# ParBLiSS/FastANI

Measured on NVIDIA H100. Metric: genome-pairs/sec (many-to-many, k=16, fragLen=3000), higher is better.
Workload: dtype u64

## Files before the change

### fastani_b200/csrc/map.cu

```cuda
#include "common.cuh"
#include "cgi_rows.hpp"
#include <algorithm>
#include <cstring>
#include <deque>

namespace bani {

static inline unsigned nblk(uint64_t n, int t = 256) { return (unsigned)((n + t - 1) / t); }

static constexpr int SU_THREADS = 128;
static constexpr int SU_CAP = 4096;

__global__ void __launch_bounds__(SU_THREADS)
sort_unique_kernel(uint32_t *fragHash, const uint32_t *segStart, int32_t F, int32_t *sCount,
                   int *smax, int *err, int minN )
{
  __shared__ uint32_t a[SU_CAP];
  __shared__ uint32_t wsum[SU_THREADS / 32];
  const int f = blockIdx.x, tid = threadIdx.x;
  const uint32_t beg = segStart[f];
  const int n = (int)(segStart[f + 1] - beg);
  if (n <= minN) return;
  if (n > SU_CAP) { if (tid == 0) { atomicExch(err, 1); sCount[f] = 0; } return; }
  if (n == 0) { if (tid == 0) sCount[f] = 0; return; }
// ... 160 lines not shown
  if (i > fragBeg) {
    const uint32_t rp = (uint32_t)a.keys[i - 1]; int32_t sp;
    if (a.recSeq[rp] == a.recSeq[ra] && l1_qual(a, i - 1, fragEnd, mh, rp, sp) && a.recWpos[rp] >= start) merged = true;
  }
  if (!merged) fl |= 1;
  bool nextMerges = false;
  if (i + 1 < fragEnd) {
    const uint32_t rn = (uint32_t)a.keys[i + 1]; int32_t sn;
    if (a.recSeq[rn] == a.recSeq[ra] && l1_qual(a, i + 1, fragEnd, mh, rn, sn) && a.recWpos[ra] >= sn) nextMerges = true;
  }
  if (!nextMerges) fl |= 2;
  return fl;
}

__global__ void l1_flag_kernel(const L1Args a, uint32_t *head)
{
  unsigned long long i = (unsigned long long)blockIdx.x * blockDim.x + threadIdx.x;
  if (i > a.N) return;
  if (i == a.N) { head[i] = 0; return; }
  int32_t start; uint32_t ra; int f;
  head[i] = l1_flags(a, i, start, ra, f) & 1u;
}

__global__ void l1_write_kernel(const L1Args a, const uint32_t *head, const uint32_t *headScan,
                                int32_t *cFrag, int32_t *cSeq, int32_t *cStart, int32_t *cEnd)
{
  unsigned long long i = (unsigned long long)blockIdx.x * blockDim.x + threadIdx.x;
  if (i >= a.N) return;
  int32_t start; uint32_t ra; int f;
  const uint32_t fl = l1_flags(a, i, start, ra, f);
  if (fl & 1) { const uint32_t c = headScan[i]; cFrag[c] = f; cSeq[c] = a.recSeq[ra]; cStart[c] = start; }
  if (fl & 2) { const uint32_t c = headScan[i] + head[i] - 1; cEnd[c] = a.recWpos[ra]; }
}

struct L2Args {
  const int32_t *cFrag, *cSeq, *cStart, *cEnd; uint32_t C;
  const uint32_t *fragHash; const uint32_t *segStart; const int32_t *sCount;
  const uint32_t *recHash; const int32_t *recWpos; const uint32_t *recLink; const uint32_t *contigRecOff;
  int fragLen, cmw, smax;
  uint8_t *scratch; size_t stride;
  int32_t *cPos, *cBest;
  int onlyFlagged;
};

__device__ __forceinline__ uint32_t lb_wpos(const int32_t *wpos, uint32_t lo, uint32_t hi, int32_t v)
{
  while (lo < hi) { uint32_t mid = (lo + hi) >> 1; if (wpos[mid] < v) lo = mid + 1; else hi = mid; }
  return lo;
}
__device__ __forceinline__ int lb_q(const uint32_t *Q, int s, uint32_t h)
{
  int lo = 0, hi = s;
  while (lo < hi) { int mid = (lo + hi) >> 1; if (Q[mid] < h) lo = mid + 1; else hi = mid; }
  return lo;
}

__global__ void __launch_bounds__(64)
l2_kernel(const L2Args a)
{
  const uint32_t slot = blockIdx.x * blockDim.x + threadIdx.x, nslots = gridDim.x * blockDim.x;
  uint16_t *gap = (uint16_t *)(a.scratch + (size_t)slot * a.stride);
  uint8_t *pres = (uint8_t *)(gap + a.smax + 2);
  for (uint32_t c = slot; c < a.C; c += nslots) {
    if (a.onlyFlagged && a.cBest[c] != -1) continue;
    const int f = a.cFrag[c];
    const int s = a.sCount[f];
    const uint32_t *Q = a.fragHash + a.segStart[f];
    const int seq = a.cSeq[c];
    const uint32_t lo = a.contigRecOff[seq], hi = a.contigRecOff[seq + 1];
    uint32_t b = lb_wpos(a.recWpos, lo, hi, a.cStart[c]);
    uint32_t e = lb_wpos(a.recWpos, lo, hi, a.recWpos[b] + a.cmw);
    const uint32_t last = lb_wpos(a.recWpos, lo, hi, a.cEnd[c] + a.fragLen);
    for (int i = 0; i <= s; i++) gap[i] = 0;
    for (int i = 0; i < s; i++) pres[i] = 0;
    int t = s, G = 0, P = 0;

    auto insert = [&](uint32_t r, uint32_t wb) {
      const uint32_t pd = a.recLink[r] >> 16;
      if (pd != 0xFFFFu && r - pd >= wb) return;
      const uint32_t h = a.recHash[r];
      const int j = lb_q(Q, s, h);
      if (j < s && Q[j] == h) { pres[j] = 1; if (j < t) P++; }
      else { gap[j]++; if (j < t) G++; while (t + G > s) { t--; G -= gap[t]; P -= pres[t]; } }
    };
    auto remove = [&](uint32_t r, uint32_t we) {
      const uint32_t nd = a.recLink[r] & 0xFFFFu;
      if (nd != 0xFFFFu && r + nd < we) return;
      const uint32_t h = a.recHash[r];
      const int j = lb_q(Q, s, h);
      if (j < s && Q[j] == h) { pres[j] = 0; if (j < t) P--; }
      else { gap[j]--; if (j < t) G--; while (t < s && t + 1 + G + (int)gap[t] <= s) { G += gap[t]; P += pres[t]; t++; } }
    };

    for (uint32_t r = b; r < e; r++) insert(r, b);
    int sw = a.recWpos[b];
    int best = 0, first = 0, lastp = 0;
    while (e < last) {
      if (P > best) { best = P; first = lastp = a.recWpos[b]; }
      else if (P == best) lastp = a.recWpos[b];
      const int d1 = a.recWpos[b + 1] - sw, d2 = a.recWpos[e] - (sw + a.cmw - 1);
      const int adv = min(d1, d2);
      sw += adv;
      const uint32_t ob = b, oe = e;
      if (adv == d1) { remove(ob, oe); b++; }
      if (adv == d2) { insert(oe, b); e++; }
    }
    a.cPos[c] = (first + lastp) / 2;
    a.cBest[c] = best;
  }
}

static constexpr int L2_SMAX = 2047;
static constexpr int L2_SHM_BUDGET = 200 * 1024;
static constexpr uint32_t EV_M = 1u, EV_D = 2u, EV_S = 4u, EV_JMASK = 0xFFE0u;
__host__ __device__ __forceinline__ uint32_t ev_rank(uint32_t j) { return j << 5; }

static constexpr int L2E_RING = 1024;
static constexpr int L2E_FLUSH_IT = 4;
static constexpr int L2E_BF_MAX = L2E_RING - 64 * L2E_FLUSH_IT - 96;

struct L2PArgs {
  const int32_t *cFrag, *cSeq, *cStart, *cEnd; uint32_t C;
  const uint32_t *fragCandOff;
  const uint32_t *fragHash; const uint32_t *segStart; const int32_t *sCount;
  const uint4 *rec; const int32_t *recWposSoA; const uint32_t *contigRecOff;
  const uint2 *rec8; const uint32_t *recLink; const uint32_t *blkMax;
  int fragLen, cmw, sLimit, shiftA, nBuckets;
  int stage;
  uint32_t *cB0, *cE0, *cLast, *cNEv, *cChunks;
  uint16_t *cMB;
  const uint32_t *cOff;
  const unsigned long long *grpOff;
  uint16_t *events;
  const uint32_t *perm; uint32_t warpBytes;
  int32_t *cPos, *cBest; unsigned long long *ctr_n2;
};

__global__ void frag_cand_off_kernel(const int32_t *cFrag, uint32_t C, int32_t F, uint32_t *fragCandOff)
{
  int f = blockIdx.x * blockDim.x + threadIdx.x;
  if (f > F) return;
  uint32_t lo = 0, hi = C;
  while (lo < hi) { uint32_t mid = (lo + hi) >> 1; if (cFrag[mid] < f) lo = mid + 1; else hi = mid; }
  fragCandOff[f] = lo;
}

__device__ __forceinline__ int32_t rec_wpos(const uint4 *rec, uint32_t i) { return (int32_t)(__ldg(&rec[i].y) & 0x7FFFFFFFu); }
__device__ __forceinline__ uint32_t lb_rec(const uint4 *rec, uint32_t lo, uint32_t hi, int32_t v)
{
  while (lo < hi) { uint32_t mid = (lo + hi) >> 1; if (rec_wpos(rec, mid) < v) lo = mid + 1; else hi = mid; }
  return lo;
}

__global__ void l2_bounds_kernel(const L2PArgs a)
{
  const uint32_t c = blockIdx.x * blockDim.x + threadIdx.x;
  unsigned long long n2 = 0;
  if (c < a.C) {
    const int seq = a.cSeq[c];
    const uint32_t lo = a.contigRecOff[seq], hi = a.contigRecOff[seq + 1];
    const uint32_t b0 = lb_wpos(a.recWposSoA, lo, hi, a.cStart[c]);
    const uint32_t e0 = lb_wpos(a.recWposSoA, b0, hi, __ldg(&a.recWposSoA[b0]) + a.cmw);
    const uint32_t last = lb_wpos(a.recWposSoA, b0, hi, a.cEnd[c] + a.fragLen);
    n2 = last - b0;
    const int s = a.sCount[a.cFrag[c]];
    uint32_t nEv = 0;
    if (e0 < last) {
      const uint32_t back = __ldg(&a.rec[last - 1].w) & 0xFFFFu;
      const uint32_t bEnd = (back > last - 1 - b0) ? b0 : last - 1 - back;
      nEv = (e0 - b0) + (last - e0) + (bEnd - b0);
    }
    a.cB0[c] = b0; a.cE0[c] = e0; a.cLast[c] = last;
    const bool fast = s >= 1 && s <= a.sLimit && nEv < (1u << 20);
    {
      uint32_t mbk = 0, mfw = 0;
      if (fast && nEv) {
        const uint32_t blk1 = (last - 1) >> 10;
        for (uint32_t blk = b0 >> 10; blk <= blk1 && mbk != 0xFFFFu; blk++) { const uint32_t v = __ldg(&a.blkMax[blk]); mbk = max(mbk, v & 0xFFFFu); mfw = max(mfw, v >> 16); }
      }
      a.cMB[c] = (uint16_t)((a.stage && mbk + mfw <= (uint32_t)L2E_BF_MAX) ? mbk : 0xFFFFu);
    }
    a.cNEv[c] = fast ? nEv : 0u;
    a.cChunks[c] = fast ? (nEv + 15) >> 4 : 0u;
    a.cBest[c] = (fast || nEv == 0) ? 0 : -1;
    a.cPos[c] = 0;
  } else if (c == a.C) a.cChunks[c] = 0;
  for (int o = 16; o; o >>= 1) n2 += __shfl_xor_sync(0xffffffffu, n2, o);
  if ((threadIdx.x & 31) == 0 && n2) atomicAdd(a.ctr_n2, n2);
}

__global__ void l2_sortkey_kernel(const uint32_t *cNEv, uint32_t C, uint32_t *key, uint32_t *val)
{
  const uint32_t c = blockIdx.x * blockDim.x + threadIdx.x;
  if (c >= C) return;
  key[c] = 0xFFFFFu - min(cNEv[c], 0xFFFFFu);
  val[c] = c;
}

__global__ void l2_group_steps_kernel(const uint32_t *cChunks, const uint32_t *perm, uint32_t C, uint32_t nGrp, uint32_t *grpSteps)
{
  const uint32_t G = blockIdx.x * blockDim.x + threadIdx.x;
  if (G > nGrp) return;
  grpSteps[G] = G < nGrp ? cChunks[perm[G * 32]] : 0u;
}
__global__ void l2_stream_base_kernel(const uint32_t *perm, const unsigned long long *grpOff, uint32_t C, uint32_t *cOff)
{
  const uint32_t g = blockIdx.x * blockDim.x + threadIdx.x;
  if (g >= C) return;
  cOff[perm[g]] = (uint32_t)(grpOff[g >> 5] * 32ull + (g & 31u));
}
__device__ __forceinline__ size_t ev_index(uint32_t base, uint32_t e) { return ((size_t)base + (size_t)(e >> 4) * 32) * 16 + (e & 15u); }

static constexpr int L2E_BUCKETS = 4096;

template <int NT>
__global__ void __launch_bounds__(NT)
l2_events_kernel(const L2PArgs a)
{
  extern __shared__ __align__(16) uint32_t smem[];
  __shared__ uint32_t s_wsum[NT / 32];
  constexpr int NW = NT / 32;
  const int f = blockIdx.x, tid = threadIdx.x, lane = tid & 31, wid = tid >> 5;
  const uint32_t c0 = a.fragCandOff[f], c1 = a.fragCandOff[f + 1];
  if (c0 == c1) return;
  const int s = a.sCount[f];
  if (s < 1 || s > a.sLimit) return;
  uint16_t *ring = reinterpret_cast<uint16_t *>(smem) + wid * L2E_RING;
  uint32_t *Q = smem + NW * (L2E_RING / 2);
  uint32_t *tab = Q + a.sLimit + 4;
  uint2 *QP = reinterpret_cast<uint2 *>(smem + ((NW * (L2E_RING / 2) + a.sLimit + 4 + L2E_BUCKETS + 4 + 1) & ~1));
  const int NB = a.nBuckets;
  {
    const uint32_t *Qg = a.fragHash + a.segStart[f];
    for (int i = tid; i < s + 3; i += NT) Q[i] = i < s ? Qg[i] : 0xFFFFFFFFu;
    for (int i = tid; i < s + 2; i += NT) QP[i] = make_uint2(i < s ? Qg[i] : 0xFFFFFFFFu, i + 1 < s ? Qg[i + 1] : 0xFFFFFFFFu);
    for (int i = tid; i <= NB; i += NT) tab[i] = 0;
    __syncthreads();
    for (int i = tid; i < s; i += NT) atomicAdd(&tab[min(Q[i] >> a.shiftA, (uint32_t)(NB - 1))], 1u);
    __syncthreads();
    const int chunk = NB / NW, cbeg = wid * chunk;
    uint32_t wt = 0;
    for (int i = lane; i < chunk; i += 32) wt += tab[cbeg + i];
#pragma unroll
    for (int o = 16; o; o >>= 1) wt += __shfl_xor_sync(0xffffffffu, wt, o);
    if (lane == 0) s_wsum[wid] = wt;
    __syncthreads();
    uint32_t carry = 0;
    for (int i = 0; i < wid; i++) carry += s_wsum[i];
    for (int i = lane; i < chunk; i += 32) {
      const uint32_t cnt = tab[cbeg + i];
      uint32_t incl = cnt;
#pragma unroll
      for (int o = 1; o < 32; o <<= 1) { const uint32_t v = __shfl_up_sync(0xffffffffu, incl, o); if (lane >= o) incl += v; }
      tab[cbeg + i] = carry + incl - cnt;
      carry += __shfl_sync(0xffffffffu, incl, 31);
    }
    if (tid == NT - 1) tab[NB] = carry;
    __syncthreads();
  }
  const uint32_t nop = ev_rank((uint32_t)s) | EV_M | EV_D;
  const uint32_t bmax = (uint32_t)(NB - 1);
  auto rank_of = [&](uint32_t h, bool &match) -> uint32_t {
    uint32_t j = tab[min(h >> a.shiftA, bmax)];
    const uint2 qq = QP[j];
    const uint32_t q0 = qq.x, q1 = qq.y;
    match = (q0 == h) || (q1 == h);
    j += (q0 < h) + (q1 < h);
    if (q1 < h) { while (Q[j] < h) j++; match = Q[j] == h; }
    return j;
  };
  for (uint32_t c = c0 + wid; c < c1; c += NW) {
    const uint32_t nEv = a.cNEv[c];
    if (nEv == 0) continue;
    const uint32_t b0 = a.cB0[c], nInit = a.cE0[c] - b0, nAll = a.cLast[c] - b0;
    const uint32_t sb = a.cOff[c];
    const uint32_t mbk = a.cMB[c];
    uint16_t *ev = a.events;
    if (mbk != 0xFFFFu) {
      const uint2 *rp = a.rec8 + b0;
      const uint32_t nIt = (nAll + 31) >> 5, nSteps = (nEv + 15) >> 4;
      uint32_t baseStep = 0;
      uint2 nxt = make_uint2(0u, 0u);
      if ((uint32_t)lane < nAll) nxt = __ldg(rp + lane);
      for (uint32_t it = 0; it < nIt; it++) {
        const uint32_t rb = it * 32 + lane;
        const uint2 rc = nxt;
        if (rb + 32 < nAll) nxt = __ldg(rp + rb + 32);
        if (rb < nAll) {
          bool match;
          const uint32_t j = rank_of(rc.x, match);
          const bool can = (int)j < s;
          const uint32_t code = ev_rank(j) | (match ? EV_M : 0u);
          const uint32_t y = rc.y, back = y & 0x3FFFu, fwd = (y >> 14) & 0x3FFFu;
          const uint32_t mb = min(back, rb);
          bool isNew = can && ((y >> 29) & 1u);
          if (can && !((y >> 29) & 1u) && rb < back) isNew = (__ldg(&a.recLink[b0 + rb]) >> 16) > rb;
          const bool sc = (rb + 1 >= nInit) && (rb + 1 != nAll);
          ring[(rb * 2 - mb) & (L2E_RING - 1)] = (uint16_t)((isNew ? (code | EV_D) : nop) | (sc ? EV_S : 0u));
          if (fwd != 0x3FFFu && rb + fwd < nAll) {
            const bool gone = can && ((y >> 30) & 1u);
            ring[(rb * 2 + fwd) & (L2E_RING - 1)] = (uint16_t)((gone ? code : nop) | (((y >> 28) & 1u) ? 0u : EV_S));
          }
        }
        const bool lastIt = it + 1 == nIt;
        if (lastIt || ((it + 1) % L2E_FLUSH_IT) == 0) {
          if (lastIt && (uint32_t)lane < ((16u - (nEv & 15u)) & 15u)) ring[(nEv + lane) & (L2E_RING - 1)] = (uint16_t)nop;
          __syncwarp();
          int fin = lastIt ? (int)nSteps : (((int)(64u * (it + 1)) - (int)mbk) >> 4);
          if (fin > (int)nSteps) fin = (int)nSteps;
          for (int k = (int)baseStep + lane; k < fin; k += 32) {
            const uint4 *src = reinterpret_cast<const uint4 *>(ring + ((k * 16) & (L2E_RING - 1)));
            uint4 *dst = reinterpret_cast<uint4 *>(ev + ((size_t)sb + (size_t)k * 32) * 16);
            const uint4 v0 = src[0], v1 = src[1];
            dst[0] = v0; dst[1] = v1;
          }
          if (fin > (int)baseStep) baseStep = (uint32_t)fin;
          __syncwarp();
        }
      }
      continue;
    }
    if (lane < ((16u - (nEv & 15u)) & 15u)) ev[ev_index(sb, nEv + lane)] = (uint16_t)nop;
    const uint4 *rp = a.rec + b0;
    uint32_t rb = lane;
    uint4 nxt = make_uint4(0, 0, 0, 0);
    if (rb < nAll) nxt = __ldg(rp + rb);
    for (; rb < nAll; rb += 32) {
      const uint4 rc = nxt;
      if (rb + 32 < nAll) nxt = __ldg(rp + rb + 32);
      bool match;
      const uint32_t j = rank_of(rc.x, match);
      const bool can = (int)j < s;
      const uint32_t code = ev_rank(j) | (match ? EV_M : 0u);
      const uint32_t pd = rc.z >> 16, nd = rc.z & 0xFFFFu, back = rc.w & 0xFFFFu, fwd = rc.w >> 16;
      const uint32_t rb2 = rb * 2;
      const uint32_t mb = min(back, rb);
      const bool isNew = can && pd > mb;
      const bool sc = (rb + 1 >= nInit) && (rb + 1 != nAll);
      ev[ev_index(sb, rb2 - mb)] = (uint16_t)((isNew ? (code | EV_D) : nop) | (sc ? EV_S : 0u));
// ... 903 lines not shown
   while (!work.empty()) {
    const QPiece &pc = *work.front();
    work.pop_front();
    const int nQc = pc.nq, q0 = pc.q0;
    const int32_t F = pc.F;
    const uint64_t T = pc.T;
    const int smax = pc.smax;
    bool split = false;
    uint64_t pp[NPATH] = {};
    auto split_in_halves = [&](PathId why) {
      if (countPaths) ctx->paths[why]++;
      int qm = 1;
      while (qm < nQc - 1 && pc.qFragOff[qm] < F / 2) qm++;
      slices.push_back(slice_piece(ctx, pc, qm, nQc)); work.push_front(slices.back().get());
      slices.push_back(slice_piece(ctx, pc, 0, qm)); work.push_front(slices.back().get());
      split = true;
    };
    View<uint32_t> fragHash; fragHash.p = pc.fragHash.p; fragHash.n = T;
    View<uint32_t> segStart; segStart.p = pc.segStart.p; segStart.n = (size_t)F + 1;
    View<int32_t> sCount; sCount.p = pc.sCount.p; sCount.n = F;
    View<int32_t> d_fragQuery; d_fragQuery.p = pc.fragQuery.p; d_fragQuery.n = F;
    View<int32_t> d_fragSeqId; d_fragSeqId.p = pc.fragSeqId.p; d_fragSeqId.n = F;

    std::vector<int32_t> hCount; std::vector<float> hIdent;
    std::vector<bani_cgi_result> hPairs;
    std::vector<bani_frag_mapping> hFrags;

    ctx->mark("piece: begin");
    if (F > 0 && ix->M > 0) {
      ctx->upload_lut(smax, pc.sCount.p, F);

      if (T > 0 && smax > 0) {
        BANI_SCRATCH(uint32_t, hitLo, T + 1);
        BANI_SCRATCH(uint32_t, hitCnt, T + 1);
        BANI_SCRATCH(unsigned long long, hitOff, T + 1);
        DevBuf<unsigned long long> walkCtr;
        if (countPaths) { walkCtr.alloc(2, st); BANI_CUDA(cudaMemsetAsync(walkCtr.p, 0, 16, st)); }
        { Stage sg(ctx, "lookup", 12.0 * T);
          const bool useFilt = ix->filt.p && pc.memberOf != ix->uid;
          lookup_kernel<<<nblk(T + 1), 256, 0, st>>>(fragHash.p, (uint32_t)T, ix->tab.p, (1u << ix->tabBits) - 1u, ix->ukeys.p, ix->uoff.p,
                                                   ix->dir.p, ix->dirBits, useFilt ? ix->filt.p : nullptr,
                                                   useFilt ? (uint32_t)((1ull << ix->filtBits) - 1ull) : 0u, hitLo.p, hitCnt.p, walkCtr.p);
          ctx->launches++;
          size_t tb = cub_scan_u64_temp(T + 1);
          BANI_SCRATCH(uint8_t, tmp, tb);
          cub_exclusive_sum_u32_to_u64(tmp.p, tb, hitCnt.p, (uint64_t *)hitOff.p, T + 1, st); }
        unsigned long long N = 0;
        BANI_CUDA(cudaMemcpyAsync(&N, hitOff.p + T, 8, cudaMemcpyDeviceToHost, st));
        if (countPaths) BANI_CUDA(cudaMemcpyAsync(pp + P_LOOKUP_WALK_SATURATED, walkCtr.p, 16, cudaMemcpyDeviceToHost, st));
        BANI_CUDA(cudaStreamSynchronize(st));
        ctx->mark("piece: lookup done");
        if (N > maxHits && nQc > 1) split_in_halves(P_PIECE_SPLIT_HITS);
        if (!split && N > 0xfffffff0ull) fail(BANI_ERR_LIMIT, "one query genome gathers more than 2^32 index hits");
        if (!split) out.ctr.hits += N;

        if (N > 0 && !split) {
          BANI_SCRATCH(uint32_t, candCount, (size_t)F + 1);
          BANI_SCRATCH(uint32_t, candOff, (size_t)F + 1);
          BANI_SCRATCH(uint32_t, fragClass, F);
          BANI_SCRATCH(uint32_t, classList, (size_t)FRAG_NCLASS * F);
          BANI_SCRATCH(uint32_t, classCount, FRAG_NCLASS + 2);
          BANI_SCRATCH(int32_t, stSeq, N);
          BANI_SCRATCH(int32_t, stStart, N);
          BANI_SCRATCH(int32_t, stEnd, N);
          const long long maxFast = std::max(0ll, std::min(ctx->flags.fragL1Max, (long long)FRAG_L1_MAX));
          uint32_t hClass[FRAG_NCLASS + 2];
          { Stage sg(ctx, "frag_l1", 12.0 * N);
            frag_classify(ctx, segStart.p, hitOff.p, F, candCount.p, fragClass.p, classCount.p, classList.p, (unsigned long long)maxFast);
            BANI_CUDA(cudaMemcpyAsync(hClass, classCount.p, sizeof hClass, cudaMemcpyDeviceToHost, st));
            BANI_CUDA(cudaStreamSynchronize(st));
            for (int i = 0; i <= FRAG_NCLASS; i++) pp[P_L1_CLASS0 + i] += hClass[i];
            FragL1Args fa; fa.segStart = segStart.p; fa.sCount = sCount.p; fa.F = F; fa.hitLo = hitLo.p; fa.hitCnt = hitCnt.p; fa.hitOff = hitOff.p;
            fa.posIdx = ix->posIdx.p; fa.recPos = ix->pos8.p; fa.minHits = ctx->d_minHits.p; fa.fragLen = fragLen;
            fa.keyBits = 1; while (fa.keyBits < 32 && (1ull << fa.keyBits) < ix->M) fa.keyBits++;
            fa.stSeq = stSeq.p; fa.stStart = stStart.p; fa.stEnd = stEnd.p; fa.candCount = candCount.p;
            frag_l1_fast(ctx, fa, classList.p, hClass); }
          if (hClass[FRAG_NCLASS] > 0) {
            BANI_SCRATCH(uint32_t, bigCnt, T + 1);
            BANI_SCRATCH(unsigned long long, bigOff, T + 1);
            mask_hits_kernel<<<nblk(T + 1), 256, 0, st>>>(segStart.p, F, (uint32_t)T, hitCnt.p, fragClass.p, bigCnt.p); ctx->launches++;
            { size_t tb = cub_scan_u64_temp(T + 1);
              BANI_SCRATCH(uint8_t, tmp, tb);
              cub_exclusive_sum_u32_to_u64(tmp.p, tb, bigCnt.p, (uint64_t *)bigOff.p, T + 1, st); }
            unsigned long long NB = 0;
            BANI_CUDA(cudaMemcpyAsync(&NB, bigOff.p + T, 8, cudaMemcpyDeviceToHost, st));
            BANI_CUDA(cudaStreamSynchronize(st));
            BANI_SCRATCH(unsigned long long, keysA, NB);
            BANI_SCRATCH(unsigned long long, keysB, NB);
            { Stage sg(ctx, "hit_gather", 12.0 * NB);
              gather_kernel<<<nblk(T), 256, 0, st>>>(segStart.p, F, (uint32_t)T, hitLo.p, bigCnt.p, bigOff.p, ix->posIdx.p, keysA.p); ctx->launches++; }
            int fbits = 1; while ((1ll << fbits) < F) fbits++;
            { Stage sg(ctx, "hit_sort", 16.0 * NB);
              size_t tb = cub_sort_keys_u64_temp(NB);
              BANI_SCRATCH(uint8_t, tmp, tb);
              cub_sort_keys_u64(tmp.p, tb, (const uint64_t *)keysA.p, (uint64_t *)keysB.p, NB, 0, 32 + fbits, st); }
            L1Args la; la.keys = keysB.p; la.N = NB; la.segStart = segStart.p; la.hitOff = bigOff.p; la.sCount = sCount.p;
            la.minHits = ctx->d_minHits.p; la.recSeq = ix->seqId.p; la.recWpos = ix->wpos.p; la.fragLen = fragLen;
            BANI_SCRATCH(uint32_t, head, NB + 1);
            BANI_SCRATCH(uint32_t, headScan, NB + 1);
            { Stage sg(ctx, "l1_flags", 8.0 * NB);
              l1_flag_kernel<<<nblk(NB + 1), 256, 0, st>>>(la, head.p);
              ctx->launches++;
              size_t tb = cub_scan_u32_temp(NB + 1);
              BANI_SCRATCH(uint8_t, tmp, tb);
              cub_exclusive_sum_u32(tmp.p, tb, head.p, headScan.p, NB + 1, st); }
            uint32_t CB = 0;
            BANI_CUDA(cudaMemcpyAsync(&CB, headScan.p + NB, 4, cudaMemcpyDeviceToHost, st));
            BANI_CUDA(cudaStreamSynchronize(st));
            if (CB > 0) {
              BANI_SCRATCH(int32_t, bFrag, CB);
              BANI_SCRATCH(int32_t, bSeq, CB);
              BANI_SCRATCH(int32_t, bStart, CB);
              BANI_SCRATCH(int32_t, bEnd, CB);
              Stage sg(ctx, "l1_write", 8.0 * NB);
              l1_write_kernel<<<nblk(NB), 256, 0, st>>>(la, head.p, headScan.p, bFrag.p, bSeq.p, bStart.p, bEnd.p); ctx->launches++;
              cand_stage(ctx, bFrag.p, bSeq.p, bStart.p, bEnd.p, CB, segStart.p, hitOff.p, stSeq.p, stStart.p, stEnd.p, candCount.p);
            }
          }
          { size_t tb = cub_scan_u32_temp((size_t)F + 1);
            BANI_SCRATCH(uint8_t, tmp, tb);
            BANI_CUDA(cudaMemsetAsync(candCount.p + F, 0, 4, st));
            cub_exclusive_sum_u32(tmp.p, tb, candCount.p, candOff.p, (size_t)F + 1, st); }
          uint32_t C = 0;
          BANI_CUDA(cudaMemcpyAsync(&C, candOff.p + F, 4, cudaMemcpyDeviceToHost, st));
          BANI_CUDA(cudaStreamSynchronize(st));
          out.ctr.candidates += C;

          if (C > 0) {
            BANI_SCRATCH(int32_t, cFrag, C);
            BANI_SCRATCH(int32_t, cSeq, C);
            BANI_SCRATCH(int32_t, cStart, C);
            BANI_SCRATCH(int32_t, cEnd, C);
            BANI_SCRATCH(int32_t, cPos, C);
            BANI_SCRATCH(int32_t, cBest, C);
            cand_compact(ctx, segStart.p, hitOff.p, F, candCount.p, candOff.p, stSeq.p, stStart.p, stEnd.p, cFrag.p, cSeq.p, cStart.p, cEnd.p);

            L2Args l2; l2.cFrag = cFrag.p; l2.cSeq = cSeq.p; l2.cStart = cStart.p; l2.cEnd = cEnd.p; l2.C = C;
            l2.fragHash = fragHash.p; l2.segStart = segStart.p; l2.sCount = sCount.p;
            l2.recHash = ix->hash.p; l2.recWpos = ix->wpos.p; l2.recLink = ix->link.p; l2.contigRecOff = ix->contigRecOff.p;
            l2.fragLen = fragLen; l2.cmw = cmw; l2.smax = smax;
            l2.stride = ((size_t)2 * (smax + 2) + smax + 15) / 16 * 16;
            const unsigned blocks = (unsigned)std::min<uint64_t>((C + 63) / 64, (uint64_t)ctx->smCount * 16);
            BANI_SCRATCH(uint8_t, scratch, (size_t)blocks * 64 * l2.stride);
            BANI_SCRATCH(unsigned long long, d_n2, 1);
            BANI_CUDA(cudaMemsetAsync(d_n2.p, 0, 8, st));
            l2.scratch = scratch.p; l2.cPos = cPos.p; l2.cBest = cBest.p; l2.onlyFlagged = 1;
            size_t idEv = (size_t)-1; double evBytes = 0;
            {
              unsigned long long totalSteps = 0;
              Stage sgb(ctx, "l2_bounds", 12.0 * C);
              BANI_SCRATCH(uint32_t, fragCandOff, (size_t)F + 1);
              frag_cand_off_kernel<<<nblk((uint64_t)F + 1), 256, 0, st>>>(cFrag.p, C, F, fragCandOff.p);
              ctx->launches++;
              L2PArgs lp; lp.cFrag = cFrag.p; lp.cSeq = cSeq.p; lp.cStart = cStart.p; lp.cEnd = cEnd.p; lp.C = C;
              lp.fragCandOff = fragCandOff.p; lp.fragHash = fragHash.p; lp.segStart = segStart.p; lp.sCount = sCount.p;
              lp.rec = ix->rec.p; lp.recWposSoA = ix->wpos.p; lp.contigRecOff = ix->contigRecOff.p; lp.fragLen = fragLen; lp.cmw = cmw;
              lp.rec8 = ix->rec8.p; lp.recLink = ix->link.p; lp.blkMax = ix->blkMax.p; lp.stage = ctx->flags.l2Stage;
              lp.sLimit = (ctx->flags.l2Fast && cmw >= 2 && ix->cmw == cmw && ix->rec8.p) ? std::min(std::min(smax, L2_SMAX), L2_SHM_BUDGET / (L2S_WARPS * 32) - 2) : 0;
              lp.nBuckets = ((uint64_t)C >= 8ull * (uint64_t)F) ? L2E_BUCKETS : 1024;
              { const int forced = ctx->flags.l2eBuckets;
                if (forced == 1024 || forced == L2E_BUCKETS) lp.nBuckets = forced; }
              { int sh = lp.nBuckets == L2E_BUCKETS ? 20 : 22; while (sh > 8 && ((uint64_t)std::max(smax, 1) * (uint64_t)w << sh) > ((1ull << 32) * (uint64_t)(L2E_BUCKETS / lp.nBuckets))) sh--; lp.shiftA = sh; }
              lp.warpBytes = (uint32_t)(std::max(lp.sLimit, 1) + 1) * 32u;
              BANI_SCRATCH(uint32_t, cB0, C);
              BANI_SCRATCH(uint32_t, cE0, C);
              BANI_SCRATCH(uint32_t, cLast, C);
              BANI_SCRATCH(uint32_t, cNEv, C);
              BANI_SCRATCH(uint32_t, cChunks, (size_t)C + 1);
              BANI_SCRATCH(uint32_t, cOff, (size_t)C + 1);
              BANI_SCRATCH(uint16_t, cMB, (size_t)C + 1);
              lp.cMB = cMB.p;
              lp.cB0 = cB0.p; lp.cE0 = cE0.p; lp.cLast = cLast.p; lp.cNEv = cNEv.p; lp.cChunks = cChunks.p; lp.cOff = cOff.p;
              lp.cPos = cPos.p; lp.cBest = cBest.p; lp.ctr_n2 = d_n2.p; lp.events = nullptr; lp.perm = nullptr;
              l2_bounds_kernel<<<nblk((uint64_t)C + 1), 256, 0, st>>>(lp); ctx->launches++;
              if (countPaths) pp[P_L2_EXACT_AT_BOUNDS] += count_exact(ctx, cBest.p, C);
              if (lp.sLimit > 0) {
                BANI_SCRATCH(uint32_t, skey, C);
                BANI_SCRATCH(uint32_t, skey2, C);
                BANI_SCRATCH(uint32_t, sval, C);
                BANI_SCRATCH(uint32_t, perm, C);
                l2_sortkey_kernel<<<nblk(C), 256, 0, st>>>(cNEv.p, C, skey.p, sval.p); ctx->launches++;
                { size_t tb = cub_sort_pairs_u32_temp(C);
                  BANI_SCRATCH(uint8_t, tmp, tb);
                  cub_sort_pairs_u32(tmp.p, tb, skey.p, skey2.p, sval.p, perm.p, C, 20, st); }
                lp.perm = perm.p;
                const uint32_t nGrp = (C + 31) / 32;
                BANI_SCRATCH(uint32_t, grpSteps, (size_t)nGrp + 1);
                BANI_SCRATCH(unsigned long long, grpOff, (size_t)nGrp + 1);
                l2_group_steps_kernel<<<nblk((uint64_t)nGrp + 1), 256, 0, st>>>(cChunks.p, perm.p, C, nGrp, grpSteps.p); ctx->launches++;
                { size_t tb = cub_scan_u64_temp((size_t)nGrp + 1);
                  BANI_SCRATCH(uint8_t, tmp, tb);
                  cub_exclusive_sum_u32_to_u64(tmp.p, tb, grpSteps.p, (uint64_t *)grpOff.p, (size_t)nGrp + 1, st); }
                unsigned long long totalGrpSteps = 0;
                BANI_CUDA(cudaMemcpyAsync(&totalGrpSteps, grpOff.p + nGrp, 8, cudaMemcpyDeviceToHost, st));
                BANI_CUDA(cudaStreamSynchronize(st));
                totalSteps = totalGrpSteps * 32;
                if ((double)totalSteps * 32.0 > evLimit && nQc > 1) {
                  out.ctr.hits -= N; out.ctr.candidates -= C;
                  split_in_halves(P_PIECE_SPLIT_EVENTS);
                  goto piece_done;
                }
                if (totalSteps > 0xfffffff0ull) fail(BANI_ERR_LIMIT, "query chunk schedules more than 2^36 window events");
                BANI_SCRATCH(uint16_t, events, (size_t)totalSteps * 16 + 64);
                lp.events = events.p; lp.grpOff = grpOff.p;
                l2_stream_base_kernel<<<nblk(C), 256, 0, st>>>(perm.p, grpOff.p, C, cOff.p); ctx->launches++;
                const int evNT = ((uint64_t)C >= 6ull * (uint64_t)F) ? 256 : ((uint64_t)C >= 3ull * (uint64_t)F) ? 128 : 64;
                if (countPaths) {
                  std::vector<uint32_t> nEv(C); std::vector<uint16_t> mb(C);
                  BANI_CUDA(cudaMemcpyAsync(nEv.data(), cNEv.p, 4 * (size_t)C, cudaMemcpyDeviceToHost, st));
                  BANI_CUDA(cudaMemcpyAsync(mb.data(), cMB.p, 2 * (size_t)C, cudaMemcpyDeviceToHost, st));
                  BANI_CUDA(cudaStreamSynchronize(st));
                  uint64_t withEv = 0, staged = 0;
                  for (uint32_t c = 0; c < C; c++) if (nEv[c]) { withEv++; staged += mb[c] != 0xFFFFu; }
                  pp[evNT == 256 ? P_L2_EVENTS_NT256 : evNT == 128 ? P_L2_EVENTS_NT128 : P_L2_EVENTS_NT64] += withEv;
                  pp[lp.nBuckets == L2E_BUCKETS ? P_L2_DIR4096 : P_L2_DIR1024] += withEv;
                  pp[P_L2_STAGED] += staged; pp[P_L2_DIRECT] += withEv - staged;
                }
                const size_t shmE = 4 * ((size_t)(evNT / 32) * (L2E_RING / 2) + (size_t)lp.sLimit + 4 + L2E_BUCKETS + 4 + 2) + 8 * ((size_t)lp.sLimit + 4) + 16;
                const size_t shmS = (size_t)L2S_WARPS * lp.warpBytes;
                if (shmE > (size_t)L2_SHM_BUDGET || shmS > (size_t)L2_SHM_BUDGET) fail(BANI_ERR_INTERNAL, "L2 shared-memory budget exceeded");
                if (ctx->first_time((const void *)l2_seq_kernel)) {
                  BANI_CUDA(cudaFuncSetAttribute(l2_events_kernel<256>, cudaFuncAttributeMaxDynamicSharedMemorySize, L2_SHM_BUDGET));
                  BANI_CUDA(cudaFuncSetAttribute(l2_events_kernel<128>, cudaFuncAttributeMaxDynamicSharedMemorySize, L2_SHM_BUDGET));
                  BANI_CUDA(cudaFuncSetAttribute(l2_events_kernel<64>, cudaFuncAttributeMaxDynamicSharedMemorySize, L2_SHM_BUDGET));
                  BANI_CUDA(cudaFuncSetAttribute(l2_seq_kernel, cudaFuncAttributeMaxDynamicSharedMemorySize, L2_SHM_BUDGET));
                  BANI_CUDA(cudaFuncSetAttribute(l2_seq_kernel, cudaFuncAttributePreferredSharedMemoryCarveout, 100));
                }
                sgb.stop();
                { Stage sg(ctx, "l2_events"); idEv = sg.id(); evBytes = 32.0 * (double)totalSteps;
                  if (evNT == 256) l2_events_kernel<256><<<F, 256, shmE, st>>>(lp);
                  else if (evNT == 128) l2_events_kernel<128><<<F, 128, shmE, st>>>(lp);
                  else l2_events_kernel<64><<<F, 64, shmE, st>>>(lp);
                  ctx->launches++; }
                { Stage sg(ctx, "l2_seq", evBytes + 16.0 * C);
                  l2_seq_kernel<<<nblk(C, L2S_WARPS * 32), L2S_WARPS * 32, shmS, st>>>(lp); ctx->launches++; }
              }
              sgb.stop();
              if (countPaths) pp[P_L2_EXACT_TOTAL] += count_exact(ctx, cBest.p, C);
              Stage sgs(ctx, "l2_exact");
              l2_kernel<<<blocks, 64, 0, st>>>(l2); ctx->launches++;
            }

            RepArgs ra; ra.cFrag = cFrag.p; ra.cSeq = cSeq.p; ra.cPos = cPos.p; ra.cBest = cBest.p; ra.C = C;
            ra.sCount = sCount.p; ra.fragSeqId = d_fragSeqId.p; ra.rowOff = ctx->d_rowOff.p; ra.ident = ctx->d_ident.p;
            ra.upper = ctx->d_upper.p; ra.pid = pid; ra.fragLen = fragLen;
            BANI_SCRATCH(uint32_t, keep, C + 1);
            BANI_SCRATCH(uint32_t, keepScan, C + 1);
            keep_flag_kernel<<<nblk(C + 1), 256, 0, st>>>(ra, keep.p);
            ctx->launches++;
            { size_t tb = cub_scan_u32_temp(C + 1);
            BANI_SCRATCH(uint8_t, tmp, tb);
              cub_exclusive_sum_u32(tmp.p, tb, keep.p, keepScan.p, C + 1, st); }
            uint32_t R = 0; unsigned long long n2 = 0;
            BANI_CUDA(cudaMemcpyAsync(&R, keepScan.p + C, 4, cudaMemcpyDeviceToHost, st));
            BANI_CUDA(cudaMemcpyAsync(&n2, d_n2.p, 8, cudaMemcpyDeviceToHost, st));
            BANI_CUDA(cudaStreamSynchronize(st));
            out.ctr.n2 += n2; out.ctr.mappings += R;
            ctx->mark("piece: L1 + L2 done");
            Stage::set_bytes(ctx, idEv, 16.0 * (double)n2 + evBytes);
            if (R > 0) {
              BANI_SCRATCH(bani_mapping, rows, R);
              DevBuf<int32_t> rFrag(R, st);
              { Stage sg(ctx, "report", 44.0 * R);
                rows_kernel<<<nblk(C), 256, 0, st>>>(ra, keep.p, keepScan.p, rows.p, rFrag.p); ctx->launches++; }
              if (wantRows) {
                size_t old = out.rows.size(); out.rows.resize(old + R);
                BANI_CUDA(cudaMemcpyAsync(out.rows.data() + old, rows.p, sizeof(bani_mapping) * (size_t)R, cudaMemcpyDeviceToHost, st));
                BANI_CUDA(cudaStreamSynchronize(st));
              }
              const bool sparse = wantCgi && (ctx->flags.cgiSparse >= 0 ? ctx->flags.cgiSparse == 1
                                                                        : (uint64_t)nQc * nG > std::max<uint64_t>(R, CGI_SPARSE_MIN_PAIRS));
              if (sparse) {
                int qBits = 0; while ((1ull << qBits) <= (uint64_t)nQc) qBits++;
                int binBits = 1; while ((1ull << binBits) < ix->totalBins) binBits++;
                if (qBits + binBits > 64) fail(BANI_ERR_LIMIT, "sparse identity reduction: %d query bits + %d bin bits exceed 64", qBits, binBits);
                CgiArgs ca; ca.rows = rows.p; ca.rFrag = rFrag.p; ca.R = R; ca.fragQuery = d_fragQuery.p;
                ca.contigGenome = ix->contigGenome.p; ca.contigBinOff = ix->contigBinOff.p; ca.fragLen = fragLen;
                ca.totalBins = ix->totalBins; ca.nGenomes = nG; ca.table = nullptr; ca.touched = nullptr; ca.qLo = 0; ca.qHi = nQc;
                BANI_SCRATCH(unsigned long long, spKey, R);
                BANI_SCRATCH(unsigned long long, spKeySorted, R);
                BANI_SCRATCH(uint32_t, spRow, R);
                BANI_SCRATCH(uint32_t, spRowSorted, R);
                BANI_SCRATCH(uint32_t, binHead, (size_t)R + 1);
                BANI_SCRATCH(uint32_t, binIdx, (size_t)R + 1);
                BANI_SCRATCH(unsigned long long, binKey, R);
                BANI_SCRATCH(uint32_t, binRow, R);
                BANI_SCRATCH(uint32_t, pairHead, (size_t)R + 1);
                BANI_SCRATCH(uint32_t, pairIdx, (size_t)R + 1);
                BANI_SCRATCH(bani_cgi_result, dPairs, R);
                Stage sg(ctx, "cgi_sparse", 150.0 * R);
                pp[P_CGI_SPARSE]++;
                cgi_sparse_key_kernel<<<nblk(R), 256, 0, st>>>(ca, binBits, nQc, spKey.p, spRow.p);
                ctx->launches++;
                { size_t tb = cub_sort_pairs_u64_u32_temp(R);
                  BANI_SCRATCH(uint8_t, tmp, tb);
                  cub_sort_pairs_u64_u32(tmp.p, tb, (const uint64_t *)spKey.p, (uint64_t *)spKeySorted.p, spRow.p, spRowSorted.p, R, qBits + binBits, st); }
                cgi_sparse_bin_head_kernel<<<nblk((uint64_t)R + 1), 256, 0, st>>>(spKeySorted.p, R, (unsigned long long)nQc << binBits, binHead.p);
                ctx->launches++;
                const size_t tbScan = cub_scan_u32_temp((size_t)R + 1);
                BANI_SCRATCH(uint8_t, scanTmp, tbScan);
                cub_exclusive_sum_u32(scanTmp.p, tbScan, binHead.p, binIdx.p, (size_t)R + 1, st);
                BANI_CUDA(cudaMemsetAsync(pairHead.p, 0, 4 * ((size_t)R + 1), st));
                cgi_sparse_bin_max_kernel<<<nblk(R), 256, 0, st>>>(ca, spKeySorted.p, spRowSorted.p, R, binBits, binHead.p, binIdx.p,
                                                                   binKey.p, binRow.p, pairHead.p);
                ctx->launches++;
                cub_exclusive_sum_u32(scanTmp.p, tbScan, pairHead.p, pairIdx.p, (size_t)R + 1, st);
                cgi_sparse_pair_kernel<<<nblk(R), 256, 0, st>>>(ca, binKey.p, binRow.p, binIdx.p + R, pairHead.p, pairIdx.p, wantFrags, dPairs.p);
                ctx->launches++;
                uint32_t nBins = 0, nPairs = 0;
                BANI_CUDA(cudaMemcpyAsync(&nBins, binIdx.p + R, 4, cudaMemcpyDeviceToHost, st));
                BANI_CUDA(cudaMemcpyAsync(&nPairs, pairIdx.p + R, 4, cudaMemcpyDeviceToHost, st));
                BANI_CUDA(cudaStreamSynchronize(st));
                if (wantFrags && nBins > 0) {
                  BANI_SCRATCH(bani_frag_mapping, dFrags, nBins);
                  cgi_frag_gather_kernel<<<nblk(nBins), 256, 0, st>>>(rows.p, binKey.p, binRow.p, nBins, dFrags.p);
                  ctx->launches++;
                  hFrags.resize(nBins);
                  BANI_CUDA(cudaMemcpyAsync(hFrags.data(), dFrags.p, sizeof(bani_frag_mapping) * (size_t)nBins, cudaMemcpyDeviceToHost, st));
                }
                hPairs.resize(nPairs);
                if (nPairs) BANI_CUDA(cudaMemcpyAsync(hPairs.data(), dPairs.p, sizeof(bani_cgi_result) * (size_t)nPairs, cudaMemcpyDeviceToHost, st));
                BANI_CUDA(cudaStreamSynchronize(st));
                ctx->mark("piece: sparse identity rows on host");
              } else if (wantCgi) {
                hCount.assign((size_t)nQc * nG, 0); hIdent.assign((size_t)nQc * nG, 0.f);
                const uint64_t needQ = std::min<uint64_t>(qMaxByTable, std::max<uint64_t>(nQc, 1));
                if (needQ > tableQ) {
// ... 102 lines not shown
```

Before: 2.119 million.

## Remap L2 bounds kernel to fragment-grouped threads ordered by contig position

```diff
diff --git a/fastani_b200/csrc/map.cu b/fastani_b200/csrc/map.cu
--- a/fastani_b200/csrc/map.cu
+++ b/fastani_b200/csrc/map.cu
@@ -336,18 +336,33 @@
   return lo;
 }
 
-__global__ void l2_bounds_kernel(const L2PArgs a)
-{
-  const uint32_t c = blockIdx.x * blockDim.x + threadIdx.x;
+__global__ void l2_frag_key_kernel(const uint32_t *fragCandOff, const int32_t *cSeq, const int32_t *cStart, int32_t F,
+                                   unsigned long long none, unsigned long long *key, uint32_t *val)
+{
+  const int f = blockIdx.x * blockDim.x + threadIdx.x;
+  if (f >= F) return;
+  const uint32_t c = fragCandOff[f];
+  key[f] = c < fragCandOff[f + 1] ? ((unsigned long long)(uint32_t)cSeq[c] << 32) | (uint32_t)cStart[c] : none;
+  val[f] = (uint32_t)f;
+}
+
+__global__ void l2_bounds_kernel(const L2PArgs a, const uint32_t *fragOrder, int32_t F, int width)
+{
+  const uint32_t gtid = blockIdx.x * blockDim.x + threadIdx.x;
+  const uint32_t g = gtid / width, sub = gtid & (width - 1);
   unsigned long long n2 = 0;
-  if (c < a.C) {
+  if (gtid == 0) a.cChunks[a.C] = 0;
+  const bool in = g < (uint32_t)F;
+  const int f = in ? (int)fragOrder[g] : 0;
+  const uint32_t c0 = in ? a.fragCandOff[f] : 0u, c1 = in ? a.fragCandOff[f + 1] : 0u;
+  for (uint32_t c = c0 + sub; c < c1; c += width) {
     const int seq = a.cSeq[c];
     const uint32_t lo = a.contigRecOff[seq], hi = a.contigRecOff[seq + 1];
     const uint32_t b0 = lb_wpos(a.recWposSoA, lo, hi, a.cStart[c]);
     const uint32_t e0 = lb_wpos(a.recWposSoA, b0, hi, __ldg(&a.recWposSoA[b0]) + a.cmw);
     const uint32_t last = lb_wpos(a.recWposSoA, b0, hi, a.cEnd[c] + a.fragLen);
-    n2 = last - b0;
-    const int s = a.sCount[a.cFrag[c]];
+    n2 += last - b0;
+    const int s = a.sCount[f];
     uint32_t nEv = 0;
     if (e0 < last) {
       const uint32_t back = __ldg(&a.rec[last - 1].w) & 0xFFFFu;
@@ -368,7 +383,7 @@
     a.cChunks[c] = fast ? (nEv + 15) >> 4 : 0u;
     a.cBest[c] = (fast || nEv == 0) ? 0 : -1;
     a.cPos[c] = 0;
-  } else if (c == a.C) a.cChunks[c] = 0;
+  }
   for (int o = 16; o; o >>= 1) n2 += __shfl_xor_sync(0xffffffffu, n2, o);
   if ((threadIdx.x & 31) == 0 && n2) atomicAdd(a.ctr_n2, n2);
 }
@@ -1578,6 +1593,16 @@
               BANI_SCRATCH(uint32_t, fragCandOff, (size_t)F + 1);
               frag_cand_off_kernel<<<nblk((uint64_t)F + 1), 256, 0, st>>>(cFrag.p, C, F, fragCandOff.p);
               ctx->launches++;
+              BANI_SCRATCH(unsigned long long, fKey, F);
+              BANI_SCRATCH(unsigned long long, fKeySorted, F);
+              BANI_SCRATCH(uint32_t, fIdx, F);
+              BANI_SCRATCH(uint32_t, fragOrder, F);
+              { int sbits = 1; while ((1ll << sbits) <= (long long)ix->nContigs) sbits++;
+                l2_frag_key_kernel<<<nblk(F), 256, 0, st>>>(fragCandOff.p, cSeq.p, cStart.p, F, (unsigned long long)ix->nContigs << 32,
+                                                            fKey.p, fIdx.p); ctx->launches++;
+                size_t tb = cub_sort_pairs_u64_u32_temp(F);
+                BANI_SCRATCH(uint8_t, tmp, tb);
+                cub_sort_pairs_u64_u32(tmp.p, tb, (const uint64_t *)fKey.p, (uint64_t *)fKeySorted.p, fIdx.p, fragOrder.p, F, 32 + sbits, st); }
               L2PArgs lp; lp.cFrag = cFrag.p; lp.cSeq = cSeq.p; lp.cStart = cStart.p; lp.cEnd = cEnd.p; lp.C = C;
               lp.fragCandOff = fragCandOff.p; lp.fragHash = fragHash.p; lp.segStart = segStart.p; lp.sCount = sCount.p;
               lp.rec = ix->rec.p; lp.recWposSoA = ix->wpos.p; lp.contigRecOff = ix->contigRecOff.p; lp.fragLen = fragLen; lp.cmw = cmw;
@@ -1598,7 +1623,8 @@
               lp.cMB = cMB.p;
               lp.cB0 = cB0.p; lp.cE0 = cE0.p; lp.cLast = cLast.p; lp.cNEv = cNEv.p; lp.cChunks = cChunks.p; lp.cOff = cOff.p;
               lp.cPos = cPos.p; lp.cBest = cBest.p; lp.ctr_n2 = d_n2.p; lp.events = nullptr; lp.perm = nullptr;
-              l2_bounds_kernel<<<nblk((uint64_t)C + 1), 256, 0, st>>>(lp); ctx->launches++;
+              { int width = 4; while (width < 32 && (uint64_t)width * (uint64_t)F < (uint64_t)C) width <<= 1;
+                l2_bounds_kernel<<<nblk((uint64_t)F * width), 256, 0, st>>>(lp, fragOrder.p, F, width); ctx->launches++; }
               if (countPaths) pp[P_L2_EXACT_AT_BOUNDS] += count_exact(ctx, cBest.p, C);
               if (lp.sLimit > 0) {
                 BANI_SCRATCH(uint32_t, skey, C);
```

After: 2.125 million, median of 6. Within noise of the previous version (+0.2%).
